# powturbo/Turbo-Range-Coder

Measured on AMD Instinct MI355X. Metric: encode+decode MB/s, order-0 static-CDF rANS, 100 MB bytes, higher is better.
Workload: dtype u32; 1 GPU; text100m: 100000000 B/GPU, static-CDF rANS, 2 states (anscdf4senc/anscdf4sdec per chunk), tables in LDS, chunk 512 B, 1 lane = 1 chunk, 64 chunks/wave; codec=anscdf4s, chunk=512, bytes_per_gpu=100000000, compressed_bytes_per_gpu=64522350, steps_in_flight=1, exchange=none

## Files before the change

turbo-range-coder_amd/csrc/trc_ans_static.hip:

```cpp
#include <stdlib.h>
#include <stdio.h>
#include <string.h>
#include "trc_io.h"
#include "trc_launch.h"

#define ENC_WAVE_LDS (TRC_SRING_BYTES)
#define ENC_TAB_LDS 4096u
#define ENC_PACE_LDS 192u
#define DEC_WAVE_LDS (TRC_SRING_BYTES)

__device__ __forceinline__ u32 ans_cur(u32 wpos)
{
    const u32 h = ~(wpos >> 1);
    return ((h & 62u) << 6) | (h & 1u);
}
__device__ __forceinline__ u32 ans_cur_wpos(u32 wpos, u32 cur)
{
    const u32 h0 = ~(wpos >> 1), h1 = ((cur >> 6) & 62u) | (cur & 1u);
    return wpos + (((h0 - h1) & 63u) << 1);
}
__device__ __forceinline__ void ans_put(u32 &st, const trc_v4u e, u32 rbase, u32 &cur)
{
    u32 t;
    asm volatile("v_cmp_ge_u32_e32 vcc, %0, %3\n\t"
                 "v_and_b32_e32 %1, %8, %1\n\t"
                 "v_lshl_add_u32 %2, %1, 1, %4\n\t"
                 "ds_write_b16 %2, %0\n\t"
                 "v_cndmask_b32_sdwa %0, %0, %0, vcc dst_sel:DWORD dst_unused:UNUSED_PAD src0_sel:DWORD src1_sel:WORD_1\n\t"
                 "v_subbrev_co_u32_e32 %1, vcc, 0, %1, vcc\n\t"
                 "v_mul_hi_u32 %2, %0, %5\n\t"
                 "v_lshrrev_b32_sdwa %2, %6, %2 dst_sel:DWORD dst_unused:UNUSED_PAD src0_sel:BYTE_3 src1_sel:DWORD\n\t"
                 "v_mul_u32_u24_e32 %2, %2, %6\n\t"
                 "v_add3_u32 %0, %0, %7, %2"
                 : "+v"(st), "+v"(cur), "=&v"(t) : "v"(e.z), "v"(rbase), "v"(e.x), "v"(e.y), "v"(e.w), "s"(0xf81u) : "vcc", "memory");
}
template <int K>
__device__ __forceinline__ u32 ans_taddr(u32 w, u32 sh)
{
    u32 a;
    if (K == 0) asm("v_lshlrev_b32_sdwa %0, %1, %2 dst_sel:DWORD dst_unused:UNUSED_PAD src0_sel:DWORD src1_sel:BYTE_0" : "=v"(a) : "v"(sh), "v"(w));
    if (K == 1) asm("v_lshlrev_b32_sdwa %0, %1, %2 dst_sel:DWORD dst_unused:UNUSED_PAD src0_sel:DWORD src1_sel:BYTE_1" : "=v"(a) : "v"(sh), "v"(w));
    if (K == 2) asm("v_lshlrev_b32_sdwa %0, %1, %2 dst_sel:DWORD dst_unused:UNUSED_PAD src0_sel:DWORD src1_sel:BYTE_2" : "=v"(a) : "v"(sh), "v"(w));
    if (K == 3) asm("v_lshlrev_b32_sdwa %0, %1, %2 dst_sel:DWORD dst_unused:UNUSED_PAD src0_sel:DWORD src1_sel:BYTE_3" : "=v"(a) : "v"(sh), "v"(w));
    return a;
}
struct EncQuad { trc_v4u e0, e1, e2, e3; };
__device__ __forceinline__ void ans_fetch4(EncQuad &q, u32 w)
{
    const u32 sh = 4u;
    q.e3 = trc_lds_read128(ans_taddr<3>(w, sh));
    q.e2 = trc_lds_read128(ans_taddr<2>(w, sh));
    q.e1 = trc_lds_read128(ans_taddr<1>(w, sh));
    q.e0 = trc_lds_read128(ans_taddr<0>(w, sh));
}
#define ANS_WAIT4(q, pending)                                                                                        \
    asm volatile("s_waitcnt lgkmcnt(" #pending ")" : "+v"(q.e0), "+v"(q.e1), "+v"(q.e2), "+v"(q.e3) :: "memory")

#ifdef TRC_ENC_PROF
__device__ unsigned long long trc_enc_wall[4 * 4096];
#endif
template <int BLOCK>
__global__ __launch_bounds__(BLOCK) void trc_ans4s_enc_kernel(
    const u8 *__restrict__ in, u64 n, u32 chunk, u32 nchunks,
    const uint4 *__restrict__ etab_g, u8 *__restrict__ scratch, u32 stride,
    u32 *__restrict__ clen, u32 *__restrict__ gsum)
{
    extern __shared__ __attribute__((aligned(16))) u8 smem[];
    const u32 tid = threadIdx.x, lane = tid & 63u, wv = tid >> 6;
#ifdef TRC_ENC_PROF
    const u64 ew0 = wall_clock64();
#endif
    u8 *wbase = smem + ENC_TAB_LDS + ENC_PACE_LDS + wv * ENC_WAVE_LDS;
    for (u32 i = tid; i < 256u; i += BLOCK) ((uint4 *)smem)[i] = etab_g[i];
    TrcPace pace; pace.init(trc_lds_addr(smem) + ENC_TAB_LDS, tid, wv);
    __syncthreads();

    WaveChunks wc;
    wc.c0 = (blockIdx.x * (BLOCK / 64) + wv) * 64u; wc.chunk = chunk; wc.nchunks = nchunks;
    wc.lastlen = (u32)(n - (u64)(nchunks - 1) * chunk);
    if (wc.c0 >= nchunks) return;
    wc.rows = nchunks - wc.c0 < 64u ? nchunks - wc.c0 : 64u;

    const bool alive = lane < wc.rows;
    const u64 amask = trc_ballot(alive);
    const u32 c = wc.c0 + lane;
    const u32 len = alive ? wc.len_of(lane) : 0u;
    QuadIn tin; tin.base = in + (u64)wc.c0 * chunk;
    StreamOut<true, false, false, true, 32u, true> so;
    so.rings = wbase;
    so.scratch = scratch; so.stride = stride; so.c0 = wc.c0; so.wpos = 0; so.nfl = 0;
    const u32 rbase = (u32)(uintptr_t)(so.rings - smem) + so.ra(lane, 0);
    const uint4 *etab1 = (const uint4 *)smem;

    const u32 S = chunk / TRC_SEG;
    const u32 top = alive ? (len - 1u) / TRC_SEG : 0u;
    const u32 toplen = len - TRC_SEG * top;
    u32 st0 = TRC_ANS_LOW, st1 = TRC_ANS_LOW;
    bool ovf = false;

    if ((S - 1u) & 1u) { tin.issue_slot<1>(wc, S - 1u); tin.issue_slot<0>(wc, S - 2u); } else tin.issue_slot<0>(wc, S - 1u);
    auto take = [&](u32 sn) {
        if (sn & 1u) tin.commit_slot<1>(); else tin.commit_slot<0>();
        if (!(sn & 1u) && sn >= 1u) {
            tin.issue_slot<1>(wc, sn - 1u);
            if (sn >= 2u) tin.issue_slot<0>(wc, sn - 2u);
        }
    };
    take(S - 1u);
#ifdef TRC_ENC_PROF
    const u64 ew1 = wall_clock64();
#endif
    for (u32 s = S - 1u;; s--) {
        if (BLOCK > 256) pace.step(S - s);
        bool act = alive && s <= top && !ovf;
        const bool ragged = act && s == top && toplen != TRC_SEG;
        if (ragged) {
            const u32 body = len & ~3u;
            const u8 *mine = in + (u64)c * chunk;
            for (u32 pos = len; pos > TRC_SEG * top;) {
                pos--;
                const uint4 e = etab1[(u32)mine[pos]];
                const trc_v4u ev = { e.x, e.y, e.z, e.w };
                u32 wn = ans_cur(so.wpos);
                if (pos >= body || !(pos & 1u)) ans_put(st0, ev, rbase, wn); else ans_put(st1, ev, rbase, wn);
                so.wpos = ans_cur_wpos(so.wpos, wn);
            }
            act = false;
        }
#pragma unroll
        for (int k = 3; k >= 0; k--) {
            if (act) {
                const uint4 v = tin.read((u32)k);
                u32 wn = ans_cur(so.wpos);
                EncQuad a, b;
                ans_fetch4(a, v.w);
                ans_fetch4(b, v.z);
                ANS_WAIT4(a, 4);
                ans_put(st1, a.e3, rbase, wn); ans_put(st0, a.e2, rbase, wn); ans_put(st1, a.e1, rbase, wn); ans_put(st0, a.e0, rbase, wn);
                ans_fetch4(a, v.y);
                ANS_WAIT4(b, 8);
                ans_put(st1, b.e3, rbase, wn); ans_put(st0, b.e2, rbase, wn); ans_put(st1, b.e1, rbase, wn); ans_put(st0, b.e0, rbase, wn);
                ans_fetch4(b, v.x);
                ANS_WAIT4(a, 8);
                ans_put(st1, a.e3, rbase, wn); ans_put(st0, a.e2, rbase, wn); ans_put(st1, a.e1, rbase, wn); ans_put(st0, a.e0, rbase, wn);
                ANS_WAIT4(b, 4);
                ans_put(st1, b.e3, rbase, wn); ans_put(st0, b.e2, rbase, wn); ans_put(st1, b.e1, rbase, wn); ans_put(st0, b.e0, rbase, wn);
                so.wpos = ans_cur_wpos(so.wpos, wn);
            }
            asm volatile("s_waitcnt lgkmcnt(0)" ::: "memory");
            if (k == 0 && s > 0) take(s - 1u);
            so.drain(false, alive, amask);
            ovf = ovf || (alive && so.wpos + 8u >= len);
            act = act && !ovf;
        }
        if (s == 0) break;
    }
#ifdef TRC_ENC_PROF
    const u64 ew2 = wall_clock64();
#endif
    u32 out_len = 0;
    if (alive) {
        if (!ovf) {
            so.put16(st0 >> 16); so.put16(st0); so.put16(st1 >> 16); so.put16(st1);
            ovf = so.wpos >= len;
        }
        out_len = ovf ? len : so.wpos;
    }
    so.drain(true, alive && !ovf);
    if (alive) clen[c] = out_len;
    const u32 gs = trc_wave_sum(out_len);
    if (lane == 0) gsum[wc.c0 >> 6] = gs;
#ifdef TRC_ENC_PROF
    if (lane == 0) { const u32 wid = (wc.c0 >> 6) & 4095u; trc_enc_wall[4 * wid] = ew0; trc_enc_wall[4 * wid + 1] = ew1; trc_enc_wall[4 * wid + 2] = ew2; trc_enc_wall[4 * wid + 3] = wall_clock64(); }
#endif
}

typedef u32 trc_v2u __attribute__((ext_vector_type(2)));
typedef __attribute__((address_space(3))) trc_v2u trc_lds_u64;
typedef __attribute__((address_space(3))) u32 trc_lds_u32;
typedef StreamInT<true> AnsStreamIn;
#define DEC_LDS_LUT   0u
#define DEC_LDS_DTAB  32768u
#define DEC_LDS_PROG  34816u
#define DEC_LDS_WAVES 34880u

__device__ __forceinline__ u32 ans_get(u32 &st, AnsStreamIn &si)
{
    const u32 slot = st & (TRC_PROB_ONE - 1);
    const u32 x = *(const trc_lds_u8 *)(uintptr_t)(DEC_LDS_LUT + slot);
    const trc_v2u e = *(const trc_lds_u64 *)(uintptr_t)(DEC_LDS_DTAB + (x << 3));
    st = __umul24(e.x, st >> TRC_PROB_BITS) + e.y + slot;
    const u32 w = si.peek16();
    const bool rn = st < TRC_ANS_LOW;
    st = rn ? (st << 16) | w : st;
    si.rpos += rn ? 2u : 0u;
    return x;
}
__device__ __forceinline__ void ans_get_pair(u32 &s0, u32 &s1, u32 &sl0, u32 &sl1, u32 lbase, u32 &hc, u32 &x0, u32 &x1, u32 sel_lo, u32 sel_hi)
{
    u32 a;
    asm("v_bfe_u32 %0, %1, 1, 5\n\tv_lshl_add_u32 %0, %0, 8, %2" : "=&v"(a) : "v"(hc), "v"(lbase));
    const u32 dw0 = *(const trc_lds_u32 *)(uintptr_t)a;
    const u32 dw1 = *(const trc_lds_u32 *)(uintptr_t)(a + 256u);
    x0 = *(const trc_lds_u8 *)(uintptr_t)(DEC_LDS_LUT + sl0);
    x1 = *(const trc_lds_u8 *)(uintptr_t)(DEC_LDS_LUT + sl1);
    const trc_v2u e0 = *(const trc_lds_u64 *)(uintptr_t)(DEC_LDS_DTAB + (x0 << 3));
    const trc_v2u e1 = *(const trc_lds_u64 *)(uintptr_t)(DEC_LDS_DTAB + (x1 << 3));
    u32 t0 = __umul24(e0.x, s0 >> TRC_PROB_BITS) + e0.y + sl0;
    u32 t1 = __umul24(e1.x, s1 >> TRC_PROB_BITS) + e1.y + sl1;
    const u32 w32 = __builtin_amdgcn_alignbit(dw1, dw0, hc << 4);
    u32 c0, c1, sl;
    u64 m1, cy;
    asm("v_cmp_gt_u32_e32 vcc, 0x8000, %[t0]\n\t"
        "v_perm_b32 %[c0], %[t0], %[w], %[slo]\n\t"
        "v_cmp_gt_u32_e64 %[m1], %[low], %[t1]\n\t"
        "v_cndmask_b32_e32 %[t0], %[t0], %[c0], vcc\n\t"
        "v_cndmask_b32_e32 %[sl], %[slo], %[shi], vcc\n\t"
        "v_addc_co_u32_e64 %[hc], %[cy], 0, %[hc], vcc\n\t"
        "v_perm_b32 %[c1], %[t1], %[w], %[sl]\n\t"
        "v_cndmask_b32_e64 %[t1], %[t1], %[c1], %[m1]\n\t"
        "v_addc_co_u32_e64 %[hc], %[cy], 0, %[hc], %[m1]\n\t"
        "v_and_b32_e32 %[n0], 0x7fff, %[t0]\n\t"
        "v_and_b32_e32 %[n1], 0x7fff, %[t1]"
        : [t0] "+v"(t0), [t1] "+v"(t1), [hc] "+v"(hc), [c0] "=&v"(c0), [c1] "=&v"(c1), [sl] "=&v"(sl), [m1] "=&s"(m1), [cy] "=&s"(cy),
          [n0] "=&v"(sl0), [n1] "=&v"(sl1)
        : [w] "v"(w32), [low] "s"(TRC_ANS_LOW), [slo] "v"(sel_lo), [shi] "v"(sel_hi) : "vcc");
    s0 = t0; s1 = t1;
}

#ifdef TRC_DEC_PROF
__device__ unsigned long long trc_dec_prof[8];
__device__ unsigned long long trc_dec_wall[2 * 4096];
#ifdef TRC_DEC_PROF_LIGHT
#define PROF_T(x) const u64 x = 0
#define PROF_ACC(acc, a, b)
#else
#define PROF_T(x) const u64 x = clock64()
#define PROF_ACC(acc, a, b) acc += (b) - (a)
#endif
#else
#define PROF_T(x)
#define PROF_ACC(acc, a, b)
#endif
__global__ __launch_bounds__(896) void trc_ans4s_dec_kernel(
    const u8 *__restrict__ payload, const u32 *__restrict__ clen, const u64 *__restrict__ goff, const u32 *__restrict__ gsum,
    u64 n, u32 chunk, u32 nchunks,
    const u8 *__restrict__ lut_g, const u32 *__restrict__ dtab_g, u8 *__restrict__ out)
{
    extern __shared__ __attribute__((aligned(16))) u8 smem[];
    if (trc_lds_addr(smem) != 0u) __builtin_trap();
    const u32 tid = threadIdx.x, lane = tid & 63u, wv = tid >> 6, BLOCK = blockDim.x;
    u8 *wbase = smem + DEC_LDS_WAVES + wv * DEC_WAVE_LDS;
    PROF_T(pt0);
#ifdef TRC_DEC_PROF
    u64 acc_p = 0, acc_f = 0, acc_s = 0;
    const u64 wall0 = wall_clock64();
#endif
    WaveChunks wc;
    wc.c0 = (blockIdx.x * (BLOCK / 64) + wv) * 64u; wc.chunk = chunk; wc.nchunks = nchunks;
    wc.lastlen = (u32)(n - (u64)(nchunks - 1) * chunk);
    const bool valid = wc.c0 < nchunks;
    wc.rows = !valid ? 0u : nchunks - wc.c0 < 64u ? nchunks - wc.c0 : 64u;
    const bool alive = lane < wc.rows;
    const u32 c = wc.c0 + lane;
    const u32 len = alive ? wc.len_of(lane) : 0u;
    const u32 cl_raw = alive ? clen[c] : 0u;
    const u64 gbase0 = valid ? trc_group_base(goff, gsum, wc.c0 >> 6) : 0ull;
    {
        uint2 *dtab = (uint2 *)(smem + DEC_LDS_DTAB);
        if (BLOCK >= 704u) {
            uint4 t0 = make_uint4(0, 0, 0, 0), t1 = t0, t2 = t0; u32 td = 0;
            t0 = ((const uint4 *)lut_g)[tid];
            t1 = ((const uint4 *)lut_g)[tid + BLOCK];
            if (tid + 2u * BLOCK < 2048u) t2 = ((const uint4 *)lut_g)[tid + 2u * BLOCK];
            if (tid < 256u) td = dtab_g[tid];
            ((uint4 *)smem)[tid] = t0; ((uint4 *)smem)[tid + BLOCK] = t1;
            if (tid + 2u * BLOCK < 2048u) ((uint4 *)smem)[tid + 2u * BLOCK] = t2;
            if (tid < 256u) dtab[tid] = make_uint2(td >> 16, 0u - (td & 0xffffu));
        } else {
            for (u32 i = tid; i < 2048; i += BLOCK) ((uint4 *)smem)[i] = ((const uint4 *)lut_g)[i];
            for (u32 i = tid; i < 256; i += BLOCK) { const u32 d = dtab_g[i]; dtab[i] = make_uint2(d >> 16, 0u - (d & 0xffffu)); }
        }
    }
    PROF_T(pt1);
    TrcPace pace; pace.init(DEC_LDS_PROG, tid, wv);

    const u32 cl = alive ? trc_min(cl_raw, len) : 0u;
    const u32 ex = trc_wave_incl_scan(cl) - cl;
    const u64 off = gbase0 + ex;
    const bool coded = alive && cl != len;

    QuadOut tout; tout.base = out + (u64)wc.c0 * chunk;
    AnsStreamIn si;
    si.rings = wbase;
    si.gbase = payload; si.soff = off + 8; si.lim = trc_sub_sat(cl, 8u);
    const u32 r0 = si.align_start(coded);
    u32 sa = 0, sb = 0;
    if (coded) { sa = trc_ld32_a2(payload + off); sb = trc_ld32_a2(payload + off + 4); }
    AnsStreamIn::Prime P;
    si.prime_issue(coded, P);
    trc_lds_barrier();
    if (!valid) return;
    si.prime_land(P, 0, coded);
    si.prime_land(P, 1, coded);
    si.rpos = r0;

    const u32 S = chunk / TRC_SEG;
    const u32 body4 = len & ~3u;
    u8 *dst = out + (u64)c * chunk;
    const u32 rbase = (u32)(uintptr_t)(si.rings - smem) + AnsStreamIn::ra(lane, 0);
    u32 sel_lo = 0x05040100u, sel_hi = 0x05040302u;
    asm volatile("" : "+v"(sel_lo), "+v"(sel_hi));
    const u64 cmask = trc_ballot(coded);
    PROF_T(pt2);
    for (u32 s = 0; s < S; s++) {
#pragma unroll
        for (int k = 0; k < 4; k++) {
            const u32 p0 = s * TRC_SEG + (u32)k * 16u;
            if (k == 0) pace.step(s * 4u + 1u);
            PROF_T(qa);
            si.period(coded && p0 < len, cmask & trc_ballot(p0 < len), k & 1);
            PROF_T(qb); PROF_ACC(acc_p, qa, qb);
            if (k == 0 && s > 0) tout.flush(wc, (s - 1u) * TRC_SEG);
            PROF_T(qc); PROF_ACC(acc_f, qb, qc);
            if (coded && p0 + 16u <= len) {
                u32 w[4];
                u32 hc = si.rpos >> 1;
                u32 slb = sb & (TRC_PROB_ONE - 1), sla = sa & (TRC_PROB_ONE - 1);
#pragma unroll
                for (int d = 0; d < 4; d++) {
                    u32 x0, x1, x2, x3;
                    ans_get_pair(sb, sa, slb, sla, rbase, hc, x0, x1, sel_lo, sel_hi);
                    ans_get_pair(sb, sa, slb, sla, rbase, hc, x2, x3, sel_lo, sel_hi);
                    w[d] = (((((x3 << 8) | x2) << 8) | x1) << 8) | x0;
                }
                si.rpos = hc << 1;
                tout.put((u32)k, make_uint4(w[0], w[1], w[2], w[3]));
                PROF_T(qd); PROF_ACC(acc_s, qc, qd);
            } else if (coded && p0 < len) {
                for (u32 pos = p0; pos < len; pos++)
                    dst[pos] = (u8)((pos >= body4 || !(pos & 1u)) ? ans_get(sb, si) : ans_get(sa, si));
            }
        }
    }
    tout.flush(wc, (S - 1u) * TRC_SEG);
    trc_wave_copy_raw(__ballot(alive && cl == len && len != 0), off, len, out + (u64)wc.c0 * chunk, chunk, payload);
#ifdef TRC_DEC_PROF
    if (lane == 0) {
#ifdef TRC_DEC_PROF_LIGHT
        const u64 pt3 = 0;
#else
        const u64 pt3 = clock64();
#endif
#ifndef TRC_DEC_PROF_LIGHT
        atomicAdd(&trc_dec_prof[0], pt1 - pt0); atomicAdd(&trc_dec_prof[1], pt2 - pt1); atomicAdd(&trc_dec_prof[2], acc_p);
        atomicAdd(&trc_dec_prof[3], acc_f); atomicAdd(&trc_dec_prof[4], acc_s); atomicAdd(&trc_dec_prof[5], pt3 - pt0); atomicAdd(&trc_dec_prof[6], 1ull);
#endif
        const u32 wid = (blockIdx.x * (BLOCK / 64) + wv) & 4095u;
        trc_dec_wall[2 * wid] = wall0; trc_dec_wall[2 * wid + 1] = wall_clock64();
    }
#endif
}

__device__ __forceinline__ u32 ans_get_half(u32 &s, u32 lbase, u32 &hc, u32 b, u32 seld)
{
    u32 a;
    asm("v_bfe_u32 %0, %1, 1, 5\n\tv_lshl_add_u32 %0, %0, 8, %2" : "=&v"(a) : "v"(hc), "v"(lbase));
    const u32 dw0 = *(const trc_lds_u32 *)(uintptr_t)a;
    const u32 dw1 = *(const trc_lds_u32 *)(uintptr_t)(a + 256u);
    const u32 sl = s & (TRC_PROB_ONE - 1);
    const u32 x = *(const trc_lds_u8 *)(uintptr_t)(DEC_LDS_LUT + sl);
    const trc_v2u e = *(const trc_lds_u64 *)(uintptr_t)(DEC_LDS_DTAB + (x << 3));
    const u32 t = __umul24(e.x, s >> TRC_PROB_BITS) + e.y + sl;
    const u32 w32 = __builtin_amdgcn_alignbit(dw1, dw0, hc << 4);
    const u32 rn = t < TRC_ANS_LOW ? 1u : 0u;
    const u32 oth = trc_quad_xor1(rn);
    const u32 sel = 0x05040100u + oth * seld;
    const u32 c = __builtin_amdgcn_perm(t, w32, sel);
    s = rn ? c : t;
    hc += rn + oth;
    return x;
}

__global__ __launch_bounds__(896) void trc_ans4s_dec2_kernel(
    const u8 *__restrict__ payload, const u32 *__restrict__ clen, const u64 *__restrict__ goff, const u32 *__restrict__ gsum,
    u64 n, u32 chunk, u32 nchunks,
    const u8 *__restrict__ lut_g, const u32 *__restrict__ dtab_g, u8 *__restrict__ out)
{
    extern __shared__ __attribute__((aligned(16))) u8 smem[];
    if (trc_lds_addr(smem) != 0u) __builtin_trap();
    const u32 tid = threadIdx.x, lane = tid & 63u, wv = tid >> 6, BLOCK = blockDim.x;
    u8 *wbase = smem + DEC_LDS_WAVES + wv * DEC_WAVE_LDS;
    {
        uint2 *dtab = (uint2 *)(smem + DEC_LDS_DTAB);
        if (BLOCK >= 704u) {
            uint4 t0 = make_uint4(0, 0, 0, 0), t1 = t0, t2 = t0; u32 td = 0;
            t0 = ((const uint4 *)lut_g)[tid];
            t1 = ((const uint4 *)lut_g)[tid + BLOCK];
            if (tid + 2u * BLOCK < 2048u) t2 = ((const uint4 *)lut_g)[tid + 2u * BLOCK];
            if (tid < 256u) td = dtab_g[tid];
            ((uint4 *)smem)[tid] = t0; ((uint4 *)smem)[tid + BLOCK] = t1;
            if (tid + 2u * BLOCK < 2048u) ((uint4 *)smem)[tid + 2u * BLOCK] = t2;
            if (tid < 256u) dtab[tid] = make_uint2(td >> 16, 0u - (td & 0xffffu));
        } else {
            for (u32 i = tid; i < 2048; i += BLOCK) ((uint4 *)smem)[i] = ((const uint4 *)lut_g)[i];
            for (u32 i = tid; i < 256; i += BLOCK) { const u32 d = dtab_g[i]; dtab[i] = make_uint2(d >> 16, 0u - (d & 0xffffu)); }
        }
    }
    __syncthreads();

    WaveChunks wc;
    wc.c0 = (blockIdx.x * (BLOCK / 64) + wv) * 32u; wc.chunk = chunk; wc.nchunks = nchunks;
    wc.lastlen = (u32)(n - (u64)(nchunks - 1) * chunk);
    if (wc.c0 >= nchunks) return;
    wc.rows = nchunks - wc.c0 < 32u ? nchunks - wc.c0 : 32u;
    const u32 g0 = wc.c0 & ~63u, cg = g0 + lane;
    const u32 lenL = cg < nchunks ? ((cg == nchunks - 1u) ? wc.lastlen : chunk) : 0u;
    const u32 clL = cg < nchunks ? trc_min(clen[cg], lenL) : 0u;
    const u32 exL = trc_wave_incl_scan(clL) - clL;
    const u64 gbase = trc_group_base(goff, gsum, wc.c0 >> 6);
    const u32 ci = lane >> 1, b = lane & 1u, srcl = (wc.c0 & 32u) + ci;
    const u32 cl = (u32)__shfl((int)clL, (int)srcl, 64), ex = (u32)__shfl((int)exL, (int)srcl, 64), len = (u32)__shfl((int)lenL, (int)srcl, 64);
    const bool alive = ci < wc.rows;
    const u32 c = wc.c0 + ci;
    const u64 off = gbase + ex;
    const bool coded = alive && cl != len;
    const bool owner = coded && b == 0u;

    QuadOut tout; tout.base = out + (u64)wc.c0 * chunk;
    AnsStreamIn si;
    si.rings = wbase;
    si.gbase = payload; si.soff = off + 8; si.lim = trc_sub_sat(cl, 8u);
    u32 st = 0;
    if (coded) st = trc_ld32_a2(payload + off + (b ? 0u : 4u));
    si.prime(owner);

    const u32 S = chunk / TRC_SEG;
    const u32 body4 = len & ~3u;
    u8 *dst = out + (u64)c * chunk;
    const u32 rbase = (u32)(uintptr_t)(si.rings - smem) + AnsStreamIn::ra(lane & ~1u, 0);
    const u32 seld = b ? 0x0202u : 0u, sh0 = 8u * b;
    u32 hc = 0;
    for (u32 s = 0; s < S; s++) {
#pragma unroll
        for (int k = 0; k < 4; k++) {
            const u32 p0 = s * TRC_SEG + (u32)k * 16u;
            si.rpos = hc << 1;
            si.period(owner && p0 < len, k & 1);
            if (k == 0 && s > 0) tout.flush(wc, (s - 1u) * TRC_SEG, true);
            const bool full = coded && p0 + 16u <= len;
            u32 w[4];
#pragma unroll
            for (int d = 0; d < 4; d++) {
                u32 m = 0;
                if (full) {
                    const u32 xa = ans_get_half(st, rbase, hc, b, seld);
                    const u32 xb = ans_get_half(st, rbase, hc, b, seld);
                    m = (xa | (xb << 16)) << sh0;
                }
                w[d] = m | trc_quad_xor1(m);
            }
            if (!full && coded && p0 < len) {
                for (u32 pos = p0; pos < len; pos++) {
                    const bool mine = ((pos < body4 && (pos & 1u)) ? 1u : 0u) == b;
                    u32 rn = 0;
                    if (mine) {
                        const u32 sl = st & (TRC_PROB_ONE - 1);
                        const u32 x = *(const trc_lds_u8 *)(uintptr_t)(DEC_LDS_LUT + sl);
                        const trc_v2u e = *(const trc_lds_u64 *)(uintptr_t)(DEC_LDS_DTAB + (x << 3));
                        const u32 t = __umul24(e.x, st >> TRC_PROB_BITS) + e.y + sl;
                        const u32 a = rbase + (((hc >> 1) & 31u) << 8) + ((hc & 1u) << 1);
                        const u32 unit = trc_ldsr16(a);
                        rn = t < TRC_ANS_LOW ? 1u : 0u;
                        st = rn ? (t << 16) | unit : t;
                        dst[pos] = (u8)x;
                    }
                    hc += rn + trc_quad_xor1(rn);
                }
            }
            tout.put((u32)k, make_uint4(w[0], w[1], w[2], w[3]));
        }
    }
    tout.flush(wc, (S - 1u) * TRC_SEG, true);
    {
        const u32 from = (lane & 31u) << 1;
        const u32 olo = (u32)__shfl((int)(u32)off, (int)from, 64), ohi = (u32)__shfl((int)(u32)(off >> 32), (int)from, 64);
        const u32 l2 = (u32)__shfl((int)len, (int)from, 64), c2 = (u32)__shfl((int)cl, (int)from, 64);
        const bool raw = lane < wc.rows && c2 == l2 && l2 != 0u;
        trc_wave_copy_raw(__ballot(raw), ((u64)ohi << 32) | olo, l2, out + (u64)wc.c0 * chunk, chunk, payload);
    }
}

void trc_launch_ans4s_enc(const TrcCodec &, const uint8_t *d_in, size_t n, uint32_t chunk, const TrcWork &w, uint32_t *d_clen, hipStream_t s)
{
    const uint4 *etab = (const uint4 *)(w.tables + TRC_TAB_ENC);
    const u32 nwaves = w.ngroups;
    static const int env_wpb = getenv("TRC_ENC_WPB") ? atoi(getenv("TRC_ENC_WPB")) : 0;
    u32 wpb = nwaves <= 12u * 256u ? 12u : 4u;
    if (nwaves < 2048) wpb = 1;
    if (env_wpb == 1 || env_wpb == 4 || env_wpb == 12) wpb = (u32)env_wpb;
    const size_t sm = ENC_TAB_LDS + ENC_PACE_LDS + wpb * ENC_WAVE_LDS;
#define TRC_ENC_CASE(W)                                                                                                 \
    TRC_RAISE_LDS_ONCE((trc_ans4s_enc_kernel<64 * W>), ENC_TAB_LDS + ENC_PACE_LDS + W * ENC_WAVE_LDS);                  \
    TRC_LAUNCH_TIMED((trc_ans4s_enc_kernel<64 * W>), dim3((nwaves + W - 1) / W), dim3(64 * W), sm, s,                   \
                     d_in, (u64)n, chunk, w.nchunks, etab, w.scratch, w.stride, d_clen, w.gsum);
    switch (wpb) {
    case 1: TRC_ENC_CASE(1) break;
    case 4: TRC_ENC_CASE(4) break;
    case 12: TRC_ENC_CASE(12) break;
    default: break;
    }
#undef TRC_ENC_CASE
#ifdef TRC_ENC_PROF
    {
        static int calls = 0;
        if (++calls % 64 == 0) {
            static unsigned long long wl[4 * 4096];
            (void)hipDeviceSynchronize();
            (void)hipMemcpyFromSymbol(wl, HIP_SYMBOL(trc_enc_wall), sizeof wl);
            const unsigned nw = nwaves < 4096u ? nwaves : 4096u;
            unsigned long long t0 = ~0ull;
            for (unsigned i = 0; i < nw; i++) if (wl[4 * i] && wl[4 * i] < t0) t0 = wl[4 * i];
            double s1[3] = { 0, 0, 0 }, s2[3] = { 0, 0, 0 }, s3[3] = { 0, 0, 0 }, mx[3] = { 0, 0, 0 }; unsigned cnt[3] = { 0, 0, 0 }; double smax = 0;
            for (unsigned i = 0; i < nw; i++) {
                const unsigned age = wpb >= 12 ? (i % wpb) / 4u : 0; if (age > 2 || !wl[4 * i]) continue;
                const double a = (wl[4 * i] - t0) * 0.01, b = (wl[4 * i + 1] - t0) * 0.01, c2 = (wl[4 * i + 2] - t0) * 0.01, d = (wl[4 * i + 3] - t0) * 0.01;
                s1[age] += b; s2[age] += c2; s3[age] += d; cnt[age]++; if (d > mx[age]) mx[age] = d; if (a > smax) smax = a;
            }
            fprintf(stderr, "[enc wall, us since the first wave's start] wpb %u, last start %.2f; by age on the SIMD: loop starts / loop ends / wave ends (mean; max end):", wpb, smax);
            for (int a = 0; a < 3; a++) if (cnt[a]) fprintf(stderr, "  %.1f / %.1f / %.1f; %.1f", s1[a] / cnt[a], s2[a] / cnt[a], s3[a] / cnt[a], mx[a]);
            fprintf(stderr, "\n");
        }
    }
#endif
}

void trc_launch_ans4s_dec(const TrcCodec &, const uint8_t *d_payload, const uint32_t *d_clen, size_t n, uint32_t chunk,
                          const TrcWork &w, uint8_t *d_out, hipStream_t s)
{
    const u8 *lut = w.tables + TRC_TAB_LUT;
    const u32 *dtab = (const u32 *)(w.tables + TRC_TAB_DEC);
    const u32 nwaves = w.ngroups;
    static const int env_pair = getenv("TRC_ANS_PAIR") ? atoi(getenv("TRC_ANS_PAIR")) : -1;
    if (env_pair == 1 || (env_pair != 0 && nwaves < 2048u)) {
        const u32 nw2 = (w.nchunks + 31u) / 32u;
        TRC_RAISE_LDS_ONCE(trc_ans4s_dec2_kernel, DEC_LDS_WAVES + 14 * DEC_WAVE_LDS);
        u32 wpb2 = (nw2 + 255u) / 256u;
        wpb2 = wpb2 < 1u ? 1u : wpb2 > 14u ? 14u : wpb2;
        TRC_LAUNCH_TIMED(trc_ans4s_dec2_kernel, dim3((nw2 + wpb2 - 1) / wpb2), dim3(64 * wpb2), DEC_LDS_WAVES + wpb2 * DEC_WAVE_LDS, s,
                           d_payload, d_clen, w.goff, w.gsum, (u64)n, chunk, w.nchunks, lut, dtab, d_out);
        return;
    }
    TRC_RAISE_LDS_ONCE(trc_ans4s_dec_kernel, DEC_LDS_WAVES + 14 * DEC_WAVE_LDS);
    u32 wpb = (nwaves + 255u) / 256u;
    wpb = wpb < 1u ? 1u : wpb > 14u ? 14u : wpb;
    if (const char *e = getenv("TRC_DEC_WPB")) { const u32 v = (u32)atoi(e); if (v >= 1 && v <= 14) wpb = v; }
    const size_t sm = DEC_LDS_WAVES + wpb * DEC_WAVE_LDS;
#ifdef TRC_DEC_PROF
#endif
    TRC_LAUNCH_TIMED(trc_ans4s_dec_kernel, dim3((nwaves + wpb - 1) / wpb), dim3(64 * wpb), sm, s,
                       d_payload, d_clen, w.goff, w.gsum, (u64)n, chunk, w.nchunks, lut, dtab, d_out);
#ifdef TRC_DEC_PROF
    {
        static int calls = 0;
        if (++calls % 64 == 0) {
            unsigned long long h[8];
            (void)hipDeviceSynchronize();
            (void)hipMemcpyFromSymbol(h, HIP_SYMBOL(trc_dec_prof), sizeof h);
            const double wv = (double)h[6];
            fprintf(stderr, "[dec prof] waves %.0f  cycles per wave: fill %.0f  dir+prime %.0f  periods %.0f  flushes %.0f  symbols %.0f  total %.0f\n",
                    wv, h[0] / wv, h[1] / wv, h[2] / wv, h[3] / wv, h[4] / wv, h[5] / wv);
            memset(h, 0, sizeof h);
            (void)hipMemcpyToSymbol(HIP_SYMBOL(trc_dec_prof), h, sizeof h);
            static unsigned long long wl[2 * 4096];
            (void)hipMemcpyFromSymbol(wl, HIP_SYMBOL(trc_dec_wall), sizeof wl);
            const unsigned nw = nwaves < 4096u ? nwaves : 4096u;
            unsigned long long t0 = ~0ull;
            for (unsigned i = 0; i < nw; i++) if (wl[2 * i] && wl[2 * i] < t0) t0 = wl[2 * i];
            double sum[3] = { 0, 0, 0 }, mx[3] = { 0, 0, 0 }, mn[3] = { 1e9, 1e9, 1e9 }; unsigned cnt[3] = { 0, 0, 0 };
            double smax = 0;
            for (unsigned i = 0; i < nw; i++) {
                const unsigned age = (i % wpb) / 4u; if (age > 2 || !wl[2 * i]) continue;
                const double e = (wl[2 * i + 1] - t0) * 0.01, st = (wl[2 * i] - t0) * 0.01;
                sum[age] += e; cnt[age]++; if (e > mx[age]) mx[age] = e; if (e < mn[age]) mn[age] = e; if (st > smax) smax = st;
            }
            fprintf(stderr, "[dec wall, us since the first wave's start] last start %.2f; wave ends by age on the SIMD (min / mean / max): first %.1f / %.1f / %.1f, second %.1f / %.1f / %.1f, third %.1f / %.1f / %.1f\n",
                    smax, mn[0], sum[0] / (cnt[0] ? cnt[0] : 1), mx[0], mn[1], sum[1] / (cnt[1] ? cnt[1] : 1), mx[1], mn[2], sum[2] / (cnt[2] ? cnt[2] : 1), mx[2]);
        }
    }
#endif
}
```

turbo-range-coder_amd/csrc/trc_io.h:

```cpp
#pragma once
#include "trc_dev.h"

#define TRC_SEG          64u
#define TRC_TILE_STRIDE  80u
#define TRC_TILE_BYTES   (64u * TRC_TILE_STRIDE)
#define TRC_SRING        128u
#define TRC_SRING_STRIDE 132u
#define TRC_SRING_BYTES  (64u * TRC_SRING_STRIDE)

__device__ __forceinline__ u32 trc_raddr(u32 lane, u32 off) { return lane * TRC_SRING_STRIDE + off; }

__device__ __forceinline__ u32 trc_mbcnt(u64 mask)
{
    return __builtin_amdgcn_mbcnt_hi((u32)(mask >> 32), __builtin_amdgcn_mbcnt_lo((u32)mask, 0u));
}

__device__ __forceinline__ u64 trc_ballot(bool p) { return __builtin_amdgcn_ballot_w64(p); }
__device__ __forceinline__ u32 trc_popc(u64 m) { u32 c; asm("s_bcnt1_i32_b64 %0, %1" : "=s"(c) : "s"(m) : "scc"); return c; }
__device__ __forceinline__ void trc_inc_in(u32 &v, u64 m) { u64 cy; asm("v_addc_co_u32_e64 %0, %1, 0, %0, %2" : "+v"(v), "=&s"(cy) : "s"(m)); }

#define TRC_GATE_SPIN_MAX (1u << 20)
#define TRC_GATE_AREA 256u
__device__ __forceinline__ bool trc_gate_wait(const u32 *gate, u32 need)
{
    u32 spins = 0;
    while (__hip_atomic_load(gate, __ATOMIC_RELAXED, __HIP_MEMORY_SCOPE_SYSTEM) < need) {
        __builtin_amdgcn_s_sleep(32);
        if (++spins > TRC_GATE_SPIN_MAX) {
            u32 *err = (u32 *)(((uintptr_t)gate & ~(uintptr_t)(TRC_GATE_AREA - 1u)) + TRC_GATE_AREA - 4u);
            __hip_atomic_store(err, 1u, __ATOMIC_RELAXED, __HIP_MEMORY_SCOPE_SYSTEM);
            return false;
        }
    }
    __builtin_amdgcn_fence(__ATOMIC_ACQUIRE, "agent");
    return true;
}

struct WaveChunks {
    u32 c0;
    u32 rows;
    u32 chunk;
    u32 lastlen;
    u32 nchunks;
    const u32 *gate = nullptr;
    u32 gate_part = 0;
    mutable u32 gate_seen = 0;
    u32 *prog = nullptr;
    u32 *prog_host = nullptr;
    u32 prog_part = 0;
    u64 skip_rows = 0;
    __device__ __forceinline__ u32 len_of(u32 row) const { return (c0 + row == nchunks - 1) ? lastlen : chunk; }
    __device__ __forceinline__ void after_flush(u32 end) const
    {
        if (!prog) return;
        if (end % prog_part != 0u && end != chunk) return;
        asm volatile("s_waitcnt vmcnt(0)" ::: "memory");
        if (trc_lane() == 0u) {
            const u32 k = (end + prog_part - 1u) / prog_part - 1u, nwaves = (nchunks + 63u) / 64u;
            const u32 old = __hip_atomic_fetch_add(prog + k, 1u, __ATOMIC_RELAXED, __HIP_MEMORY_SCOPE_AGENT);
            if (old == nwaves - 1u) __hip_atomic_store(prog_host + k, 1u, __ATOMIC_RELEASE, __HIP_MEMORY_SCOPE_SYSTEM);
        }
    }
    __device__ __forceinline__ void wait_for(u32 segoff) const
    {
        if (!gate) return;
        const u32 need = segoff / gate_part + 1u;
        if (need > gate_seen) gate_seen = trc_gate_wait(gate, need) ? need : ~0u;
    }
};

struct TileIn {
    u8 *tile;
    const u8 *base;
    uint4 r[4];
    __device__ __forceinline__ void issue(const WaveChunks &w, u32 segoff)
    {
        const u32 lane = trc_lane(), part = (lane & 3u) << 4;
#pragma unroll
        for (int j = 0; j < 4; j++) {
            u32 row = (u32)j * 16u + (lane >> 2);
            row = row < w.rows ? row : w.rows - 1;
            const u32 so = segoff < w.len_of(row) ? segoff : 0u;
            r[j] = trc_ld16_nt(base + (size_t)row * w.chunk + so + part);
        }
    }
    __device__ __forceinline__ void commit()
    {
        const u32 lane = trc_lane(), part = (lane & 3u) << 4;
#pragma unroll
        for (int j = 0; j < 4; j++)
            *(uint4 *)(tile + ((u32)j * 16u + (lane >> 2)) * TRC_TILE_STRIDE + part) = r[j];
    }
    __device__ __forceinline__ uint4 read(u32 k) const { return *(const uint4 *)(tile + trc_lane() * TRC_TILE_STRIDE + (k << 4)); }
};

__device__ __forceinline__ u32 trc_quad_xor1(u32 v) { return (u32)__builtin_amdgcn_update_dpp(0, (int)v, 0xB1, 0xf, 0xf, false); }
#define TRC_QT_PAIR(PERM, KEEPX, KEEPY, A0, A1, A2, A3, B0, B1, B2, B3, X0, X1, X2, X3, Y0, Y1, Y2, Y3)                             \
    asm volatile("s_mov_b64 vcc, %[kx]\n\ts_nop 0\n\t"                                                                              \
        "v_cndmask_b32_dpp %[a0], %[y0], %[x0], vcc " PERM " row_mask:0xf bank_mask:0xf\n\t"                                        \
        "v_mov_b32_dpp %[b0], %[x0] " PERM " row_mask:0xf bank_mask:0xf\n\t"                                                        \
        "v_cndmask_b32_e64 %[b0], %[b0], %[y0], %[ky]\n\t"                                                                          \
        "v_cndmask_b32_dpp %[a1], %[y1], %[x1], vcc " PERM " row_mask:0xf bank_mask:0xf\n\t"                                        \
        "v_mov_b32_dpp %[b1], %[x1] " PERM " row_mask:0xf bank_mask:0xf\n\t"                                                        \
        "v_cndmask_b32_e64 %[b1], %[b1], %[y1], %[ky]\n\t"                                                                          \
        "v_cndmask_b32_dpp %[a2], %[y2], %[x2], vcc " PERM " row_mask:0xf bank_mask:0xf\n\t"                                        \
        "v_mov_b32_dpp %[b2], %[x2] " PERM " row_mask:0xf bank_mask:0xf\n\t"                                                        \
        "v_cndmask_b32_e64 %[b2], %[b2], %[y2], %[ky]\n\t"                                                                          \
        "v_cndmask_b32_dpp %[a3], %[y3], %[x3], vcc " PERM " row_mask:0xf bank_mask:0xf\n\t"                                        \
        "v_mov_b32_dpp %[b3], %[x3] " PERM " row_mask:0xf bank_mask:0xf\n\t"                                                        \
        "v_cndmask_b32_e64 %[b3], %[b3], %[y3], %[ky]"                                                                              \
        : [a0] "=&v"(A0), [a1] "=&v"(A1), [a2] "=&v"(A2), [a3] "=&v"(A3), [b0] "=&v"(B0), [b1] "=&v"(B1), [b2] "=&v"(B2), [b3] "=&v"(B3) \
        : [kx] "s"(KEEPX), [ky] "s"(KEEPY), [x0] "v"(X0), [x1] "v"(X1), [x2] "v"(X2), [x3] "v"(X3),                                 \
          [y0] "v"(Y0), [y1] "v"(Y1), [y2] "v"(Y2), [y3] "v"(Y3) : "vcc")
__device__ __forceinline__ void trc_quad_transpose_dpp(u32 (&m)[4][4])
{
    const u64 even = 0x5555555555555555ull, odd = 0xAAAAAAAAAAAAAAAAull, lo2 = 0x3333333333333333ull, hi2 = 0xCCCCCCCCCCCCCCCCull;
    u32 a[4][4];
    TRC_QT_PAIR("quad_perm:[1,0,3,2]", even, odd, a[0][0], a[0][1], a[0][2], a[0][3], a[1][0], a[1][1], a[1][2], a[1][3],
                m[0][0], m[0][1], m[0][2], m[0][3], m[1][0], m[1][1], m[1][2], m[1][3]);
    TRC_QT_PAIR("quad_perm:[1,0,3,2]", even, odd, a[2][0], a[2][1], a[2][2], a[2][3], a[3][0], a[3][1], a[3][2], a[3][3],
                m[2][0], m[2][1], m[2][2], m[2][3], m[3][0], m[3][1], m[3][2], m[3][3]);
    TRC_QT_PAIR("quad_perm:[2,3,0,1]", lo2, hi2, m[0][0], m[0][1], m[0][2], m[0][3], m[2][0], m[2][1], m[2][2], m[2][3],
                a[0][0], a[0][1], a[0][2], a[0][3], a[2][0], a[2][1], a[2][2], a[2][3]);
    TRC_QT_PAIR("quad_perm:[2,3,0,1]", lo2, hi2, m[1][0], m[1][1], m[1][2], m[1][3], m[3][0], m[3][1], m[3][2], m[3][3],
                a[1][0], a[1][1], a[1][2], a[1][3], a[3][0], a[3][1], a[3][2], a[3][3]);
}
__device__ __forceinline__ void trc_quad_transpose(u32 (&m)[4][4]) { trc_quad_transpose_dpp(m); }

struct QuadIn {
    const u8 *base;
    uint4 r[4];
    uint4 r2[4];
    uint4 p[4];
    __device__ __forceinline__ void issue(const WaveChunks &w, u32 segoff, bool pair = false)
    {
        const u32 lane = trc_lane(), part = (lane & 3u) << 4;
        w.wait_for(segoff);
#pragma unroll
        for (int j = 0; j < 4; j++) {
            u32 row = (lane & ~3u) + (u32)j;
            if (pair) row >>= 1;
            row = row < w.rows ? row : w.rows - 1;
            const u32 so = segoff < w.len_of(row) ? segoff : 0u;
            r[j] = trc_ld16_nt(base + (size_t)row * w.chunk + so + part);
        }
    }
    __device__ __forceinline__ void commit()
    {
        u32 m[4][4];
#pragma unroll
        for (int j = 0; j < 4; j++) { m[j][0] = r[j].x; m[j][1] = r[j].y; m[j][2] = r[j].z; m[j][3] = r[j].w; }
        trc_quad_transpose(m);
#pragma unroll
        for (int k = 0; k < 4; k++) p[k] = make_uint4(m[k][0], m[k][1], m[k][2], m[k][3]);
    }
    __device__ __forceinline__ uint4 read(u32 k) const { return p[k]; }

    template <int ODD>
    __device__ __forceinline__ void issue_slot(const WaveChunks &w, u32 s)
    {
        const u32 lane = trc_lane(), part = (lane & 3u) << 4, segoff = s * TRC_SEG;
#pragma unroll
        for (int j = 0; j < 4; j++) {
            u32 row = (lane & ~3u) + (u32)j;
            row = row < w.rows ? row : w.rows - 1;
            const u32 so = segoff < w.len_of(row) ? segoff : 0u;
            const uint4 v = trc_ld16_nt(base + (size_t)row * w.chunk + so + part);
            if (ODD) r[j] = v; else r2[j] = v;
        }
    }
    template <int ODD>
    __device__ __forceinline__ void commit_slot()
    {
        u32 m[4][4];
#pragma unroll
        for (int j = 0; j < 4; j++) {
            const uint4 v = ODD ? r[j] : r2[j];
            m[j][0] = v.x; m[j][1] = v.y; m[j][2] = v.z; m[j][3] = v.w;
        }
        trc_quad_transpose(m);
#pragma unroll
        for (int k = 0; k < 4; k++) p[k] = make_uint4(m[k][0], m[k][1], m[k][2], m[k][3]);
    }
};

struct QuadOut {
    u8 *base;
    uint4 p[4];
    __device__ __forceinline__ void put(u32 k, uint4 v) { p[k] = v; }
    __device__ __forceinline__ void flush(const WaveChunks &w, u32 segoff, bool pair = false)
    {
        const u32 lane = trc_lane();
        u32 m[4][4];
#pragma unroll
        for (int k = 0; k < 4; k++) { m[k][0] = p[k].x; m[k][1] = p[k].y; m[k][2] = p[k].z; m[k][3] = p[k].w; }
        trc_quad_transpose(m);
        const u32 part = (lane & 3u) << 4;
#pragma unroll
        for (int j = 0; j < 4; j++) {
            if (pair && (j & 1)) continue;
            const u32 vrow = (lane & ~3u) + (u32)j, row = pair ? vrow >> 1 : vrow;
            if (row < w.rows && segoff + part + 16u <= w.len_of(row) && !((w.skip_rows >> row) & 1ull)) {
                u8 *const a = base + (size_t)row * w.chunk + segoff + part;
                const uint4 v = make_uint4(m[j][0], m[j][1], m[j][2], m[j][3]);
                if (w.prog) trc_st16_sys(a, v); else trc_st16_nt(a, v);
            }
        }
        w.after_flush(segoff + TRC_SEG);
    }
};

template <bool DOWN, bool PAIR = false, bool QUAD = false, bool WT = false, u32 G = 0u, bool IL = false>
struct StreamOut {
    static_assert(G == 0u || (!QUAD && G + TRC_SEG <= TRC_SRING - 2u), "full-round drains: one lane per ring, and a ready lane must not be urgent by itself");
    static_assert(!IL || (!PAIR && !QUAD), "the interleaved ring: one lane per ring");
    static __device__ __forceinline__ u32 ra(u32 row, u32 off)
    {
        return IL ? ((off >> 2) << 8) + (row << 2) + (off & 2u) : trc_raddr(row, off);
    }
    u8 *rings;
    u8 *scratch;
    u32 stride;
    u32 c0;
    u8 *scratch_b;
    u32 stride_b;
    __device__ __forceinline__ u32 my_row() const { return PAIR ? trc_lane() >> 1 : QUAD ? trc_lane() >> 2 : trc_lane(); }
    __device__ __forceinline__ u32 ring_row() const { return QUAD ? trc_lane() >> 2 : trc_lane(); }
    __device__ __forceinline__ void put16_at(bool take, u32 p, u32 v)
    {
        if (take) *(u16 *)(rings + ra(ring_row(), roff16(p))) = (u16)v;
    }
    __device__ __forceinline__ u32 my_stride() const { return (PAIR && (trc_lane() & 1u)) ? stride_b : stride; }
    __device__ __forceinline__ u8 *my_region() const
    {
        return (PAIR && (trc_lane() & 1u)) ? scratch_b + (size_t)(c0 + my_row()) * stride_b : scratch + (size_t)(c0 + my_row()) * stride;
    }
    u32 wpos;
    u32 nfl;

    __device__ __forceinline__ u32 roff16(u32 p) const { return DOWN ? ((0u - (p + 2u)) & (TRC_SRING - 1)) : (p & (TRC_SRING - 1)); }
    __device__ __forceinline__ u32 roff32(u32 p) const { return DOWN ? ((0u - (p + 4u)) & (TRC_SRING - 1)) : (p & (TRC_SRING - 1)); }
    __device__ __forceinline__ void put16_if(bool take, u32 v)
    {
        *(u16 *)(rings + ra(trc_lane(), roff16(wpos))) = (u16)v;
        wpos += take ? 2u : 0u;
    }
    __device__ __forceinline__ void put32_if(bool take, u32 v)
    {
        static_assert(!IL, "the interleaved ring takes 16-bit units only");
        *(u32 *)(rings + trc_raddr(trc_lane(), roff32(wpos))) = v;
        wpos += take ? 4u : 0u;
    }
    __device__ __forceinline__ void put16(u32 v) { *(u16 *)(rings + ra(trc_lane(), roff16(wpos))) = (u16)v; wpos += 2; }
    __device__ __forceinline__ void put32(u32 v) { static_assert(!IL, "the interleaved ring takes 16-bit units only"); *(u32 *)(rings + trc_raddr(trc_lane(), roff32(wpos))) = v; wpos += 4; }

    __device__ __forceinline__ u32 pending() const { return wpos - TRC_SEG * nfl; }
    __device__ __forceinline__ void self_drain()
    {
        static_assert(!IL, "the interleaved ring is drained by the wave");
        const u32 ro = DOWN ? ((0u - TRC_SEG * (nfl + 1u)) & (TRC_SRING - 1)) : ((TRC_SEG * nfl) & (TRC_SRING - 1));
        u8 *reg = my_region();
        u8 *d = DOWN ? reg + my_stride() - (size_t)TRC_SEG * (nfl + 1u) : reg + (size_t)TRC_SEG * nfl;
        for (u32 i = 0; i < 16; i++) ((u32 *)d)[i] = *(const u32 *)(rings + trc_raddr(trc_lane(), ro + 4u * i));
        nfl++;
    }
    __device__ __forceinline__ void put32_slow(u32 v)
    {
        if (pending() + 4u > TRC_SRING - 4u && (size_t)TRC_SEG * (nfl + 2u) <= my_stride()) self_drain();
        put32(v);
    }
    __device__ __forceinline__ void put16_slow(u32 v)
    {
        if (pending() + 2u > TRC_SRING - 4u && (size_t)TRC_SEG * (nfl + 2u) <= my_stride()) self_drain();
        put16(v);
    }

    __device__ __forceinline__ void drain(bool final, bool alive) { drain(final, alive, trc_ballot(alive)); }
    __device__ __forceinline__ void drain(bool final, bool alive, u64 alive_mask)
    {
        const u32 lane = trc_lane();
        const u32 rw = trc_lds_addr(rings);
        const bool able = alive && (!QUAD || (lane & 3u) == 0u);
        const u64 amask = alive_mask & (QUAD ? 0x1111111111111111ull : ~0ull);
        auto full = [&]() { return final ? wpos > TRC_SEG * nfl : pending() >= TRC_SEG; };
        u64 mask = amask & trc_ballot(full());
        while (mask) {
            const u32 cnt = G != 0u ? trc_popc(mask) : (u32)__popcll(mask);
            if (G != 0u && !final && cnt < 16u) {
                if (!(amask & trc_ballot(pending() > TRC_SRING - 2u - G))) break;
            }
            const u32 rank = trc_mbcnt(mask);
            const u64 pmask = mask & trc_ballot(rank < 16u);
            const bool pick = able && full() && rank < 16u;
            const u32 ro = DOWN ? ((0u - TRC_SEG * (nfl + 1u)) & (TRC_SRING - 1)) : ((TRC_SEG * nfl) & (TRC_SRING - 1));
            const u32 from = rw + ra(ring_row(), ro);
            const u32 to = (my_row() * my_stride() + (DOWN ? my_stride() - TRC_SEG * (nfl + 1u) : TRC_SEG * nfl)) | (PAIR ? lane & 1u : 0u);
            const int dst = (int)((pick ? rank << 2 : 1u) << 2);
            const u32 from_l = (u32)__builtin_amdgcn_ds_permute(dst, (int)from), to_l = (u32)__builtin_amdgcn_ds_permute(dst, (int)to);
            const u32 from_q = (u32)__builtin_amdgcn_update_dpp(0, (int)from_l, 0x00, 0xf, 0xf, false);
            const u32 to_q = (u32)__builtin_amdgcn_update_dpp(0, (int)to_l, 0x00, 0xf, 0xf, false);
            const u32 q = lane >> 2, part = (lane & 3u) << 4;
            if (q < cnt && q < 16u) {
                typedef __attribute__((address_space(3))) u32 lds_u32;
                const u32 a = from_q + (IL ? part << 6 : part), st = IL ? 256u : 4u;
                const u32 s0 = *(const lds_u32 *)(uintptr_t)a, s1 = *(const lds_u32 *)(uintptr_t)(a + st);
                const u32 s2 = *(const lds_u32 *)(uintptr_t)(a + 2u * st), s3 = *(const lds_u32 *)(uintptr_t)(a + 3u * st);
                u8 *base = (PAIR && (to_q & 1u)) ? scratch_b + (size_t)c0 * stride_b : scratch + (size_t)c0 * stride;
if constexpr (WT) {
                    const trc_v4u vv = { s0, s1, s2, s3 };
                    u8 *pp = base + (to_q & ~1u) + part;
                    asm volatile("global_store_dwordx4 %0, %1, off sc1\n\ts_nop 1" :: "v"(pp), "v"(vv) : "memory");
                } else
                    *(uint4 *)(base + (to_q & ~1u) + part) = make_uint4(s0, s1, s2, s3);
            }
            trc_inc_in(nfl, pmask);
            mask = amask & trc_ballot(full());
        }
        if (QUAD) nfl = (u32)__builtin_amdgcn_update_dpp(0, (int)nfl, 0x00, 0xf, 0xf, false);
    }
};

template <bool IL>
struct StreamInT {
    static __device__ __forceinline__ u32 ra(u32 lane, u32 off)
    {
        return IL ? ((off >> 2) << 8) + (lane << 2) + (off & 3u) : trc_raddr(lane, off);
    }
    u8 *rings;
    const u8 *gbase;
    u64 soff;
    u64 wbase;
    u32 srel;
    u32 lim;
    u32 rpos;
    u32 lbytes;
    u32 infl;
    u32 rw;
    u64 mineA, mineB;
    uint4 hvA, hvB; u32 hdA, hdB; bool hokA, hokB;

    __device__ __forceinline__ u32 align_start(bool on)
    {
        const u32 r0 = on ? trc_min((u32)(((uintptr_t)gbase + soff) & 63u), soff < 62u ? (u32)soff : 62u) & ~1u : 0u;
        soff -= r0; lim += r0;
        return r0;
    }
    __device__ __forceinline__ u32 peek16() const { return *(const u16 *)(rings + ra(trc_lane(), rpos & (TRC_SRING - 1))); }
    __device__ __forceinline__ u32 peek32() const { return *(const u32 *)(rings + ra(trc_lane(), rpos & (TRC_SRING - 1))); }
    __device__ __forceinline__ u32 avail() const { return lbytes - rpos; }
    __device__ __forceinline__ void skip_if(bool take) { rpos += take ? 4u : 0u; }

    __device__ __forceinline__ void prime(bool alive)
    {
        rpos = 0; lbytes = 0; infl = 0; mineA = mineB = 0; hokA = hokB = false;
        rw = trc_lds_addr(rings);
        {
            const u32 blo = (u32)__builtin_amdgcn_readfirstlane((int)(u32)soff), bhi = (u32)__builtin_amdgcn_readfirstlane((int)(u32)(soff >> 32));
            wbase = ((u64)bhi << 32) | blo;
            srel = (u32)(soff - wbase);
        }
        hvA = hvB = make_uint4(0, 0, 0, 0); hdA = hdB = 0;
        const u64 amask = __ballot(alive);
        if (!amask) return;
        const u32 lane = trc_lane(), q = lane >> 2, part = lane & 3u;
        uint4 v[8];
        u32 at[4];
#pragma unroll
        for (u32 g = 0; g < 4; g++) {
            const u32 j = g * 16u + q;
            const u32 sr = (u32)__shfl((int)srel, (int)j, 64);
            at[g] = ((amask >> j) & 1u) ? rw + ra(j, 0) + part * PIECE_STEP : ~0u;
            const u8 *src = gbase + wbase + sr + (part << 4);
            v[2 * g] = make_uint4(0, 0, 0, 0); v[2 * g + 1] = v[2 * g];
            if (at[g] != ~0u) { v[2 * g] = trc_ld16_a2(src); v[2 * g + 1] = trc_ld16_a2(src + TRC_SEG); }
        }
#pragma unroll
        for (u32 g = 0; g < 4; g++)
            if (at[g] != ~0u) {
                put_piece(at[g] | (part == 0u ? 1u : 0u), v[2 * g]);
                put_piece(at[g] + (ra(0, TRC_SEG) - ra(0, 0)), v[2 * g + 1]);
            }
        if (alive) lbytes = TRC_SRING;
    }
    struct Prime { uint4 v[8]; u32 at[4]; };
    __device__ __forceinline__ void prime_issue(bool alive, Prime &P)
    {
        rpos = 0; lbytes = 0; infl = 0; mineA = mineB = 0; hokA = hokB = false;
        rw = trc_lds_addr(rings);
        {
            const u32 blo = (u32)__builtin_amdgcn_readfirstlane((int)(u32)soff), bhi = (u32)__builtin_amdgcn_readfirstlane((int)(u32)(soff >> 32));
            wbase = ((u64)bhi << 32) | blo;
            srel = (u32)(soff - wbase);
        }
        hvA = hvB = make_uint4(0, 0, 0, 0); hdA = hdB = 0;
        const u64 amask = __ballot(alive);
        const u32 lane = trc_lane(), q = lane >> 2, part = lane & 3u;
        const u8 *src[4];
#pragma unroll
        for (u32 g = 0; g < 4; g++) {
            const u32 j = g * 16u + q;
            const u32 sr = (u32)__shfl((int)srel, (int)j, 64);
            const bool on = (amask >> j) & 1u;
            P.at[g] = on ? rw + ra(j, 0) + part * PIECE_STEP : ~0u;
            src[g] = gbase + wbase + (on ? sr : 0u) + (part << 4);
        }
#pragma unroll
        for (u32 g = 0; g < 4; g++) P.v[2 * g] = trc_ld16_a2(src[g]);
#pragma unroll
        for (u32 g = 0; g < 4; g++) P.v[2 * g + 1] = trc_ld16_a2(src[g] + TRC_SEG);
    }
    __device__ __forceinline__ void prime_land(const Prime &P, int half, bool alive)
    {
        const u32 part = trc_lane() & 3u;
#pragma unroll
        for (u32 g = 0; g < 4; g++)
            if (P.at[g] != ~0u) {
                if (half == 0) put_piece(P.at[g] | (part == 0u ? 1u : 0u), P.v[2 * g]);
                else put_piece(P.at[g] + (ra(0, TRC_SEG) - ra(0, 0)), P.v[2 * g + 1]);
            }
        if (alive) { if (half == 0) { lbytes = TRC_SEG; infl = 1; } else { lbytes = TRC_SRING; infl -= 1; } }
    }
    static constexpr u32 PIECE_STEP = IL ? 1024u : 16u;
    static constexpr u32 GUARD_OFF = IL ? 8192u : TRC_SRING;
    typedef __attribute__((address_space(3))) u32 lds_u32;
    __device__ __forceinline__ void put_piece(u32 hd, uint4 v)
    {
        const u32 a = hd & ~3u;
        if (IL) {
            *(lds_u32 *)(uintptr_t)a = v.x;          *(lds_u32 *)(uintptr_t)(a + 256u) = v.y;
            *(lds_u32 *)(uintptr_t)(a + 512u) = v.z; *(lds_u32 *)(uintptr_t)(a + 768u) = v.w;
        } else {
            *(lds_u32 *)(uintptr_t)a = v.x;        *(lds_u32 *)(uintptr_t)(a + 4u) = v.y;
            *(lds_u32 *)(uintptr_t)(a + 8u) = v.z; *(lds_u32 *)(uintptr_t)(a + 12u) = v.w;
        }
        if (hd & 1u) *(lds_u32 *)(uintptr_t)(a + GUARD_OFF) = v.x;
    }
    __device__ __forceinline__ void landed(u64 m)
    {
        u32 t; u64 cy;
        asm("v_cndmask_b32_e64 %[t], 0, 64, %[m]\n\t"
            "v_subb_co_u32_e64 %[fl], %[cy], %[fl], 0, %[m]\n\t"
            "v_add_u32_e32 %[lb], %[lb], %[t]"
            : [t] "=&v"(t), [fl] "+v"(infl), [lb] "+v"(lbytes), [cy] "=&s"(cy) : [m] "s"(m));
    }
    __device__ __forceinline__ void commit(int par)
    {
        if (par == 0) {
            if (hokA) { put_piece(hdA, hvA); hokA = false; }
            landed(mineA); mineA = 0;
        } else {
            if (hokB) { put_piece(hdB, hvB); hokB = false; }
            landed(mineB); mineB = 0;
        }
    }
    __device__ __forceinline__ void refill(bool alive, u64 amask, int par)
    {
        const u32 lane = trc_lane();
        const bool room = avail() + TRC_SEG * infl <= TRC_SEG;
        const u64 mask = amask & trc_ballot(room);
        if (!mask) return;
        const u32 rank = trc_mbcnt(mask);
        const u64 pmask = mask & trc_ballot(rank < 16u);
        const bool pick = alive && room && rank < 16u;
        const u32 cnt = (u32)__popcll(mask);
        const u32 nx = lbytes + TRC_SEG * infl;
        const u32 ro = nx & (TRC_SRING - 1);
        const u32 src = srel + trc_min(nx, lim);
        const u32 slot = (rw + ra(lane, ro)) | (ro == 0u ? 1u : 0u);
        const int dst = (int)((pick ? rank << 2 : 1u) << 2);
        const u32 src_l = (u32)__builtin_amdgcn_ds_permute(dst, (int)src), slot_l = (u32)__builtin_amdgcn_ds_permute(dst, (int)slot);
        const u32 src_q = (u32)__builtin_amdgcn_update_dpp(0, (int)src_l, 0x00, 0xf, 0xf, false);
        const u32 slot_q = (u32)__builtin_amdgcn_update_dpp(0, (int)slot_l, 0x00, 0xf, 0xf, false);
        const u32 q = lane >> 2, part = lane & 3u;
        if (q < cnt && q < 16u) {
            const uint4 v = trc_ld16_a2(gbase + wbase + src_q + (part << 4));
            const u32 dd = ((slot_q & ~1u) + part * PIECE_STEP) | (part == 0u ? slot_q & 1u : 0u);
            if (par == 0) { hvA = v; hdA = dd; hokA = true; } else { hvB = v; hdB = dd; hokB = true; }
        }
        trc_inc_in(infl, pmask);
        if (par == 0) mineA = pmask; else mineB = pmask;
    }
    __device__ __forceinline__ void sync_refill(bool alive, u64 amask, int par)
    {
        commit(par ^ 1);
        while (amask & trc_ballot(avail() <= TRC_SEG)) {
            refill(alive, amask, 0);
            commit(0);
        }
    }
    __device__ __forceinline__ void period(bool alive, u64 amask, int par)
    {
        commit(par);
        if (amask & trc_ballot(avail() < 36u)) sync_refill(alive, amask, par);
        refill(alive, amask, par);
    }
    __device__ __forceinline__ void period(bool alive, int par) { period(alive, trc_ballot(alive), par); }
};
typedef StreamInT<false> StreamIn;
```

Baseline: 740,700 MB/s.

## Use per-lane 16-byte piece prefetch stream for rANS decode input

Adds a LaneStreamIn that keeps its own request cursor per lane and issues up to two 16-byte global loads per period into registers, then lands them into the LDS ring one period later (double-buffered A/B). The static rANS decoder switches to it in place of the shared StreamInT refill. The goal is to decouple each lane's input fetch from wave-wide refill and hide global latency across periods. In exchange it holds four extra uint4 values in registers per lane, which raises register pressure, and it adds divergent branches and a synchronous fallback path.

```diff
diff --git a/turbo-range-coder_amd/csrc/trc_ans_static.hip b/turbo-range-coder_amd/csrc/trc_ans_static.hip
--- a/turbo-range-coder_amd/csrc/trc_ans_static.hip
+++ b/turbo-range-coder_amd/csrc/trc_ans_static.hip
@@ -179,6 +179,7 @@
 typedef __attribute__((address_space(3))) trc_v2u trc_lds_u64;
 typedef __attribute__((address_space(3))) u32 trc_lds_u32;
 typedef StreamInT<true> AnsStreamIn;
+typedef LaneStreamIn AnsLaneIn;
 #define DEC_LDS_LUT   0u
 #define DEC_LDS_DTAB  32768u
 #define DEC_LDS_PROG  34816u
@@ -291,7 +292,7 @@
     const bool coded = alive && cl != len;
 
     QuadOut tout; tout.base = out + (u64)wc.c0 * chunk;
-    AnsStreamIn si;
+    AnsLaneIn si;
     si.rings = wbase;
     si.gbase = payload; si.soff = off + 8; si.lim = trc_sub_sat(cl, 8u);
     const u32 r0 = si.align_start(coded);
@@ -304,6 +305,7 @@
     si.prime_land(P, 0, coded);
     si.prime_land(P, 1, coded);
     si.rpos = r0;
+    si.start();
 
     const u32 S = chunk / TRC_SEG;
     const u32 body4 = len & ~3u;
diff --git a/turbo-range-coder_amd/csrc/trc_io.h b/turbo-range-coder_amd/csrc/trc_io.h
--- a/turbo-range-coder_amd/csrc/trc_io.h
+++ b/turbo-range-coder_amd/csrc/trc_io.h
@@ -497,3 +497,64 @@
     __device__ __forceinline__ void period(bool alive, int par) { period(alive, trc_ballot(alive), par); }
 };
 typedef StreamInT<false> StreamIn;
+
+struct LaneStreamIn : StreamInT<true> {
+    static constexpr u32 PIECE = 16u;
+    u32 req;
+    u32 dueA, dueB;
+    uint4 pA, pB;
+    uint4 qA, qB;
+    __device__ __forceinline__ void start()
+    {
+        req = lbytes; dueA = dueB = 0;
+        pA = pB = qA = qB = make_uint4(0, 0, 0, 0);
+    }
+    __device__ __forceinline__ uint4 fetch() const { return trc_ld16_a2(gbase + wbase + (srel + trc_min(req, lim))); }
+    __device__ __forceinline__ void land(uint4 v)
+    {
+        const u32 ro = lbytes & (TRC_SRING - 1);
+        const u32 a = rw + (trc_lane() << 2) + (ro << 6);
+        *(lds_u32 *)(uintptr_t)a = v.x;          *(lds_u32 *)(uintptr_t)(a + 256u) = v.y;
+        *(lds_u32 *)(uintptr_t)(a + 512u) = v.z; *(lds_u32 *)(uintptr_t)(a + 768u) = v.w;
+        if (ro == 0u) *(lds_u32 *)(uintptr_t)(a + GUARD_OFF) = v.x;
+        lbytes += PIECE;
+    }
+    __device__ __forceinline__ void commit(int par)
+    {
+        const u32 due = par == 0 ? dueA : dueB;
+        if (lbytes < due) land(par == 0 ? pA : pB);
+        if (trc_ballot(lbytes < due)) {
+            if (lbytes < due) land(par == 0 ? qA : qB);
+        }
+    }
+    __device__ __forceinline__ void request(bool alive, u64 amask, int par)
+    {
+        const u32 t = req - rpos;
+        if (alive && t <= TRC_SRING - PIECE) {
+            const uint4 v = fetch();
+            if (par == 0) pA = v; else pB = v;
+            req += PIECE;
+        }
+        if (amask & trc_ballot(t <= TRC_SRING - 2u * PIECE)) {
+            if (alive && t <= TRC_SRING - 2u * PIECE) {
+                const uint4 v = fetch();
+                if (par == 0) qA = v; else qB = v;
+                req += PIECE;
+            }
+        }
+        if (par == 0) dueA = req; else dueB = req;
+    }
+    __device__ __forceinline__ void sync_refill(bool alive, u64 amask, int par)
+    {
+        commit(par ^ 1);
+        while (amask & trc_ballot(avail() <= TRC_SEG)) {
+            if (alive && avail() <= TRC_SRING - PIECE) { land(fetch()); req += PIECE; }
+        }
+    }
+    __device__ __forceinline__ void period(bool alive, u64 amask, int par)
+    {
+        commit(par);
+        if (amask & trc_ballot(avail() < 36u)) sync_refill(alive, amask, par);
+        request(alive, amask, par);
+    }
+};
```

New measurement: 754,800 MB/s, median of 6. 1.9% higher.
